# lior1990/hp-vae-gan

Hardware: AMD Instinct MI355X
Metric: train iters/sec per pyramid scale, air_balloons 13f@144p (higher is better)
Workload: dtype f32

## Files before the change

hp-vae-gan_amd/csrc/conv_mfma.hip:

```cpp
#include "hpvg_common.h"
#include "hpvg_host.h"
#include "hpvg.h"
#include <stdlib.h>

namespace {

__device__ const float g_zero_word[16] = {0.f, 0.f, 0.f, 0.f, 0.f, 0.f, 0.f, 0.f, 0.f, 0.f, 0.f, 0.f, 0.f, 0.f, 0.f, 0.f};
constexpr long HPVG_ZERO_PLANE_FLOATS = 1L << 18;
__device__ float g_zero_plane[HPVG_ZERO_PLANE_FLOATS];

#ifdef HPVG_TRACE
__device__ unsigned long long g_trace[8192 * 4];
__device__ unsigned long long g_phase[8192 * 4];
#define HPVG_PH(i) { unsigned long long now_ = __builtin_readcyclecounter(); ph_a[i] += now_ - ph_t; ph_t = now_; }
#define HPVG_PH_INIT unsigned long long ph_t = __builtin_readcyclecounter(); unsigned long long ph_a[4] = {0, 0, 0, 0};
#define HPVG_PH_END if (threadIdx.x == 0) { for (int i_ = 0; i_ < 4; ++i_) g_phase[4 * blockIdx.x + i_] = ph_a[i_]; }
#define HPVG_TRACE_BEGIN unsigned long long tr_t0 = wall_clock64(); unsigned long long tr_c0 = __builtin_readcyclecounter();
#define HPVG_TRACE_END                                                              \
  if (threadIdx.x == 0 && blockIdx.x + gridDim.x * (blockIdx.y + gridDim.y * blockIdx.z) < 8192) { \
    unsigned long long* tr = g_trace + 4 * (blockIdx.x + gridDim.x * (blockIdx.y + gridDim.y * blockIdx.z)); \
    tr[0] = tr_t0;                                                                  \
    tr[1] = wall_clock64();                                                         \
    tr[2] = __builtin_amdgcn_s_getreg((31 << 11) | 4);                              \
    tr[3] = (__builtin_amdgcn_s_getreg((31 << 11) | 20) & 0xF) | ((__builtin_readcyclecounter() - tr_c0) << 8); \
// ... 655 lines not shown
#pragma unroll
            for (int nt = 0; nt < NT; ++nt) acc[jj][nt] = __builtin_amdgcn_mfma_f32_32x32x2f32(v, Bf[j][nt], acc[jj][nt], 0, 0, 0);
          }
        }
      }
    };
    load_chunk(av[0], bv[0], 0);
    for (int s0 = 0; s0 < ksteps; s0 += 2 * KC) {
      load_chunk(av[1], bv[1], s0 + KC);
      __builtin_amdgcn_sched_barrier(0);
      mma_chunk(av[0], bv[0], s0);
      __builtin_amdgcn_sched_barrier(0);
      load_chunk(av[0], bv[0], s0 + 2 * KC);
      __builtin_amdgcn_sched_barrier(0);
      mma_chunk(av[1], bv[1], s0 + KC);
      __builtin_amdgcn_sched_barrier(0);
    }
#pragma unroll
    for (int nt = 0; nt < NT; ++nt) {
      const int n = nt * 32 + l31;
      if (n < CO9) {
#pragma unroll
        for (int jj = 0; jj < JB; ++jj)
#pragma unroll
          for (int e = 0; e < 16; ++e) P[n * pitch + GP * grp + JB * ((e & 3) + 8 * (e >> 2) + 4 * half) + jj] = acc[jj][nt][e];
      }
    }
  }
  __syncthreads();

  const int ob = g.ob[band], on = g.on[band];
  const int nout = g.Th * on;
  for (int idx = tid; idx < nout; idx += 256) {
    const int hh = idx / on, cc = idx - hh * on;
    const int gh = h0 + hh, gw = ob + cc;
    if (gh >= a.H) continue;
    const long sp = (long)t * HW + (long)gh * a.W + gw;
    for (int o = 0; o < a.Cout; ++o) {
      float v = 0.f;
#pragma unroll
      for (int dh = 0; dh < 3; ++dh)
#pragma unroll
        for (int dw = 0; dw < 3; ++dw) {
          const int gwt = gw + dw - 1;
          if (gwt >= 0 && gwt < a.W) v += P[(o * 9 + dh * 3 + dw) * pitch + (hh + dh) * RS + (gwt - wsb)];
        }
      if (a.bias) v += a.bias[o];
      if (a.out_lrelu) v = hpvg_lrelu(v);
      a.y[((long)b * a.Cout + o) * a.T * HW + sp] = v;
    }
  }
}

__global__ void conv_pack_narrow_kernel(const float* __restrict__ w, const float* __restrict__ inv_scale, float* __restrict__ wn,
                                        int Cin_k, int Cout_k, int KT, int NT, int ksteps, int transpose_flip, long total) {
  const long idx = (long)blockIdx.x * blockDim.x + threadIdx.x;
  if (idx >= total) return;
  const int lane = idx & 63;
  long r = idx >> 6;
  const int nt = r % NT;
  const int s = (int)(r / NT);
  const int k = (lane >> 5) * ksteps + s;
  const int n = nt * 32 + (lane & 31);
  const int c = k / KT, dt = k - c * KT;
  const int o = n / 9, tap = dt * 9 + (n - o * 9);
  const int taps = KT * 9;
  float val = 0.f;
  if (o < Cout_k && c < Cin_k) {
    if (!transpose_flip) val = w[((long)o * Cin_k + c) * taps + tap];
    else val = w[((long)c * Cout_k + o) * taps + (taps - 1 - tap)];
    if (inv_scale) val *= inv_scale[0];
  }
  wn[idx] = val;
}

__global__ void conv_pack_kernel(const float* __restrict__ w, const float* __restrict__ inv_scale, float* __restrict__ wp,
                                 int Cin_k, int Cout_k, int taps, int CC, int nchunk, int mbtot, int transpose_flip,
                                 long total_direct, long total) {
  const long idx = (long)blockIdx.x * blockDim.x + threadIdx.x;
  if (idx >= total) return;
  if (idx >= total_direct) {
    const long iw = idx - total_direct;
    const long nw1 = ((long)((Cin_k + WINO_CC - 1) / WINO_CC) * (taps / 9) * 3 * 4 + 4) * mbtot * 64 * (WINO_CC / 2);
    float val = iw < nw1 ? wino_pack_value(w, iw, Cin_k, Cout_k, taps / 9, (Cin_k + WINO_CC - 1) / WINO_CC, mbtot, transpose_flip)
                         : wino2_pack_value(w, iw - nw1, Cin_k, Cout_k, (Cin_k + 3) / 4, 2 * ((mbtot + 1) / 2), transpose_flip);
    if (inv_scale) val *= inv_scale[0];
    wp[idx] = val;
    return;
  }
  const int CP = CC / 2;
  long r = idx;
  const int cp = r % CP; r /= CP;
  const int lane = r % 64; r /= 64;
  const int mb = r % mbtot; r /= mbtot;
  const int tap = r % taps; r /= taps;
  const int ch = (int)r;
  float val = 0.f;
  if (ch < nchunk) {
    const int o = mb * 32 + (lane & 31);
    const int c = ch * CC + 2 * cp + (lane >> 5);
    if (o < Cout_k && c < Cin_k) {
      if (!transpose_flip) val = w[((long)o * Cin_k + c) * taps + tap];
      else val = w[((long)c * Cout_k + o) * taps + (taps - 1 - tap)];
      if (inv_scale) val *= inv_scale[0];
    }
  }
  wp[idx] = val;
}

struct PackBatchArgs {
  const float* w[HPVG_PACK_BATCH_MAX];
  float* wp[HPVG_PACK_BATCH_MAX];
  int flip[HPVG_PACK_BATCH_MAX];
};
__global__ void conv_pack_batch_kernel(const PackBatchArgs a, int C, int taps, int CC, int nchunk, int mbtot, long total_direct,
                                       long total) {
  const long idx = (long)blockIdx.x * blockDim.x + threadIdx.x;
  if (idx >= total) return;
  const int it = blockIdx.y;
  const float* __restrict__ w = a.w[it];
  const int transpose_flip = a.flip[it];
  if (idx >= total_direct) {
    const long iw = idx - total_direct;
    const long nw1 = ((long)((C + WINO_CC - 1) / WINO_CC) * (taps / 9) * 3 * 4 + 4) * mbtot * 64 * (WINO_CC / 2);
    a.wp[it][idx] = iw < nw1 ? wino_pack_value(w, iw, C, C, taps / 9, (C + WINO_CC - 1) / WINO_CC, mbtot, transpose_flip)
                             : wino2_pack_value(w, iw - nw1, C, C, (C + 3) / 4, 2 * ((mbtot + 1) / 2), transpose_flip);
    return;
  }
  const int CP = CC / 2;
  long r = idx;
  const int cp = r % CP; r /= CP;
  const int lane = r % 64; r /= 64;
  const int mb = r % mbtot; r /= mbtot;
  const int tap = r % taps; r /= taps;
  const int ch = (int)r;
  float val = 0.f;
  if (ch < nchunk) {
    const int o = mb * 32 + (lane & 31);
    const int c = ch * CC + 2 * cp + (lane >> 5);
    if (o < C && c < C) {
      if (!transpose_flip) val = w[((long)o * C + c) * taps + tap];
      else val = w[((long)c * C + o) * taps + (taps - 1 - tap)];
    }
  }
  a.wp[it][idx] = val;
}

struct CShape { int B, Cin, Cout, T, H, W, KT; };
inline int conv_check(const CShape& c) {
  if (c.B < 1 || c.Cin < 1 || c.Cout < 1 || c.T < 1 || c.H < 1 || c.W < 1) return HPVG_ERR_ARG;
  return c.KT == 1 || c.KT == 3 ? HPVG_OK : HPVG_ERR_UNSUPPORTED;
}

struct CKnobs {
  bool sk_off;
  bool narrow2_off;
  bool w2r;
  bool w2d_off;
  bool w2_split_off;
  int stagger;
  int only_nb, only_mb, only_ntw;
  int env_wino;
  int wino;
  long min_pos;
  int stg;
  int w2d;
  int gen;
};
CKnobs& cknobs() {
  static CKnobs knobs = [] {
    auto num = [](const char* name, long dflt) { const char* e = getenv(name); return e ? atol(e) : dflt; };
    CKnobs k{};
    k.sk_off = num("HPVG_CONV_SK", 1) == 0;
    k.narrow2_off = num("HPVG_NARROW2", 1) == 0;
    k.w2r = num("HPVG_WINO2R", 1) != 0;
    k.w2d_off = num("HPVG_WINO2D", 1) == 0;
    k.w2_split_off = num("HPVG_W2_SPLIT", 1) == 0;
    k.stagger = (int)num("HPVG_WINO_STAGGER", 0);
    k.only_nb = (int)num("HPVG_PLAN_NB", 0);
    k.only_mb = (int)num("HPVG_PLAN_MB", 0);
    k.only_ntw = (int)num("HPVG_PLAN_NTW", 0);
    k.wino = k.env_wino = (int)num("HPVG_WINO", 1);
    k.min_pos = num("HPVG_WINO_MIN", -1);
    const long stg = num("HPVG_WINO_STG", 0);
    k.stg = stg == 1 || stg == 2 ? (int)stg : 0;
    return k;
  }();
  return knobs;
}

inline int conv_cc(int Cin) { return Cin <= 4 ? 4 : 8; }
inline bool conv_is_narrow(int Cin, int Cout) { return Cout <= 4 && Cin > 4; }
inline bool conv_is_wino(const CKnobs& k, int Cin, int Cout) { return k.env_wino != 0 && Cin >= 8 && Cout > 32; }
inline bool conv_is_wino2d(const CKnobs& k, int Cin, int Cout, int KT) { return !k.w2d_off && KT == 3 && conv_is_wino(k, Cin, Cout); }

inline size_t direct_pack_floats(int Cin, int Cout, int KT) {
  const int CC = conv_cc(Cin);
  const int nchunk = hpvg_cdiv(Cin, CC);
  const int mbtot = hpvg_cdiv(Cout, 32);
  const size_t per_tap = (size_t)mbtot * 64 * (CC / 2);
  return ((size_t)nchunk * KT * 9 + 2) * per_tap;
}
size_t wpack_floats(int Cin, int Cout, int KT, bool with2d) {
  const CKnobs& k = cknobs();
  if (conv_is_narrow(Cin, Cout)) return (size_t)hpvg_cdiv(Cin * KT, 2) * hpvg_cdiv(9 * Cout, 32) * 64;
  return direct_pack_floats(Cin, Cout, KT) + (conv_is_wino(k, Cin, Cout) ? wino_pack_floats(Cin, Cout, KT) : 0) +
         (with2d && conv_is_wino2d(k, Cin, Cout, KT) ? wino2_pack_floats(Cin, Cout) : 0);
}

struct Plan {
  int Th, Tw, RS, PL, L, qstride, nrange, ntw, nblocks, NB, MB, gridy, nj;
  size_t lds;
  int stg;
};

constexpr long CONV_SLOTS = 2L * HPVG_NUM_CU;
inline long conv_slots(int MB, int NB) { return (long)HPVG_CONV_WGS(MB, NB) * HPVG_NUM_CU; }

inline double conv_cost(bool streamk, long ntl, int nchunk, long slots, double mfma_paired, double mfma_alone, double stage_us,
                        int blocks) {
  if (!streamk) {
    const long per_cu = (ntl + HPVG_NUM_CU - 1) / HPVG_NUM_CU;
    const double tile_paired = nchunk * (mfma_paired + 6.0 + stage_us) + 0.4 * blocks;
    const double tile_alone = nchunk * (mfma_alone + 2.0 + stage_us) + 0.4 * blocks;
    return (double)(per_cu / 2) * tile_paired + (double)(per_cu & 1) * tile_alone + 1e-4 * (double)ntl;
  }
  const long items_tot = ntl * nchunk;
// ... 193 lines not shown
  const int GP = 32 * JB;
  double best = 1e300;
  bool found = false;
  auto bands = [&](int RS, Narrow2Geom* q) -> int {
    int nb = 0, o = 0;
    while (o < W) {
      if (nb == 16) return 0;
      int n, ws;
      if (nb == 0) { n = (RS == W) ? W : RS - 1; ws = 0; }
      else if (W - o <= RS - 1) { n = W - o; ws = W - RS; }
      else { n = RS - 2; ws = o - 1; }
      if (n < 1) return 0;
      if (q) { q->ws[nb] = ws; q->ob[nb] = o; q->on[nb] = n; }
      o += n;
      ++nb;
    }
    return nb;
  };
  for (int RS = 4; RS <= 256 && RS <= W; RS += 4) {
    const int nb = bands(RS, nullptr);
    if (nb == 0) continue;
    for (int Th = 1; Th <= H; ++Th) {
      const int nth = hpvg_cdiv(H, Th);
      if (Th != hpvg_cdiv(H, nth)) continue;
      const int npos = (Th + 2) * RS;
      const int G = hpvg_cdiv(npos, GP);
      if (G > 16) break;
      const int pitch = (G * GP) | 1;
      if ((size_t)(9 * Cout) * pitch * sizeof(float) > 76 * 1024) break;
      const long nt = (long)B * T * nth * nb;
      const double rounds = hpvg_cdiv(G, 4);
      const double waves = nt <= 2L * HPVG_NUM_CU ? 1.0 : (double)nt / (2.0 * HPVG_NUM_CU);
      const double cost = waves * (rounds * GP + 30.0);
      if (cost < best) {
        best = cost;
        found = true;
        Narrow2Geom q{};
        q.RS = RS; q.Th = Th; q.nth = nth; q.nb = nb; q.npos = npos; q.G = G; q.pitch = pitch;
        bands(RS, &q);
        *out = q;
        *ntiles = nt;
      }
    }
  }
  if (!found) return false;
  for (int k = 0; k < out->nb; ++k) {
    const int lo = out->ob[k] - 1 < 0 ? 0 : out->ob[k] - 1;
    const int hi = out->ob[k] + out->on[k] > W - 1 ? W - 1 : out->ob[k] + out->on[k];
    if (out->on[k] < 0 || lo < out->ws[k] || hi >= out->ws[k] + out->RS) return false;
  }
  return true;
}

struct CPlans {
  Plan direct[2], wino[2];
  W2Geom w2;
  Narrow2Geom n2;
  long n2_tiles;
  bool n2_ok;
};
const CPlans& conv_plans(const CKnobs& k, const CShape& c) {
  return memo_lookup<CPlans>(k.gen, c.B, c.Cin, c.Cout, c.T, c.H, c.W, c.KT, [&] {
    CPlans pl{};
    if (conv_is_narrow(c.Cin, c.Cout)) {
      pl.direct[0] = pl.direct[1] = plan_narrow_search(c);
      pl.n2_ok = plan_narrow2(c.B, c.Cin, c.Cout, c.T, c.H, c.W, c.KT, &pl.n2, &pl.n2_tiles);
      return pl;
    }
    for (int sk = 0; sk < 2; ++sk) {
      pl.direct[sk] = plan_conv_search(k, c, sk != 0);
      if (conv_is_wino(k, c.Cin, c.Cout)) pl.wino[sk] = plan_wino_search(k, c, sk != 0);
    }
    pl.w2 = wino2d_geom(k, c);
    return pl;
  });
}

inline int conv_ntiles(const CShape& c, const Plan& p) { return c.B * c.T * p.nrange * p.ntw * p.gridy; }
inline int conv_sk_grid(const CShape& c, const Plan& p) {
  const long items = (long)conv_ntiles(c, p) * hpvg_cdiv(c.Cin, conv_cc(c.Cin));
  const long slots = conv_slots(p.MB, p.NB);
  return (int)(items < slots ? items : slots);
}
inline size_t conv_sk_ws_bytes(const CShape& c, const Plan& p) {
  return p.L ? (size_t)conv_sk_grid(c, p) * 2 * p.MB * p.NB * 16 * 256 * sizeof(float) : 0;
}

inline bool conv_use_wino(const CKnobs& k, const CShape& c, bool prologue) {
  if (prologue || !conv_is_wino(k, c.Cin, c.Cout) || k.wino == 0) return false;
  if (k.wino == 2) return true;
  const long min_pos = k.min_pos >= 0 ? k.min_pos : (c.KT == 3 ? 0L : 24000L);
  return (long)c.B * c.T * c.H * c.W >= min_pos;
}
inline bool conv_use_wino2d(const CKnobs& k, const W2Geom& q) {
  if (!q.ok || k.w2d == 1) return false;
  if (k.w2d == 2) return true;
  const long rounds = (q.ntl + HPVG_NUM_CU - 1) / HPVG_NUM_CU;
  if (rounds == 1) return q.ntl * 2 >= HPVG_NUM_CU;
  return (long)q.ntl * 10 >= 6L * rounds * HPVG_NUM_CU;
}

struct CDecision {
  int kind;
  int narrow_gen;
  const CPlans* plans;
  const Plan* plan;
  bool streamk;
  int ntl, S;
  size_t ws_bytes;
};
CDecision conv_decide(const CShape& c, bool prologue, bool fp32_out_mask, const void* ws, size_t ws_bytes) {
  const CKnobs& k = cknobs();
  CDecision d{};
  const CPlans& pl = conv_plans(k, c);
  d.plans = &pl;
  if (conv_is_narrow(c.Cin, c.Cout)) {
    d.kind = 3;
    d.plan = &pl.direct[0];
    d.narrow_gen = !k.narrow2_off && !prologue && !fp32_out_mask && pl.n2_ok ? 2 : 1;
    d.ntl = d.S = conv_ntiles(c, *d.plan);
    return d;
  }
  bool wino = conv_use_wino(k, c, prologue);
  if (wino && conv_use_wino2d(k, pl.w2) && !fp32_out_mask) {
    d.kind = 2;
    d.ntl = pl.w2.ntl;
    d.S = d.ntl < HPVG_NUM_CU ? d.ntl : HPVG_NUM_CU;
    return d;
  }
  d.streamk = !k.sk_off && ws != nullptr;
  if (wino && pl.wino[d.streamk].L == 0) wino = false;
  const Plan* both = wino ? pl.wino : pl.direct;
  if (d.streamk && ws_bytes < conv_sk_ws_bytes(c, both[1])) d.streamk = false;
  d.kind = wino ? 1 : 0;
  d.plan = &both[d.streamk];
  d.ntl = conv_ntiles(c, *d.plan);
  d.S = d.streamk ? conv_sk_grid(c, *d.plan) : d.ntl;
  d.ws_bytes = d.streamk ? conv_sk_ws_bytes(c, *d.plan) : 0;
  return d;
}
inline CDecision conv_decide_query(const CShape& c) { return conv_decide(c, false, false, &c, ~(size_t)0); }

struct CCall {
  const float* x; const float* wp; const float* bias;
  const float* in_scale; const float* in_shift; int in_lrelu;
  float* y; int out_lrelu;
  const float* out_mask; const unsigned* mask_bits; unsigned* bits_out;
  void* ws; size_t ws_bytes;
  CShape c;
  hipStream_t s;
};

ConvFwdArgs conv_args(const CCall& q, const CDecision& d, int stagger) {
  const CShape& c = q.c;
  const Plan& p = *d.plan;
  ConvFwdArgs a{};
  a.x = q.x; a.bias = q.bias; a.in_scale = q.in_scale; a.in_shift = q.in_shift; a.mask = q.out_mask; a.y = q.y;
  a.wp = d.kind == 1 ? q.wp + direct_pack_floats(c.Cin, c.Cout, c.KT) : q.wp;
  a.mask_bits = q.mask_bits; a.bits_out = q.bits_out;
  a.B = c.B; a.Cin = c.Cin; a.Cout = c.Cout; a.T = c.T; a.H = c.H; a.W = c.W;
  a.Th = p.Th; a.Tw = p.Tw; a.RS = p.RS; a.PL = p.PL; a.L = p.L; a.qstride = p.qstride; a.nrange = p.nrange; a.ntw = p.ntw; a.nblocks = p.nblocks;
  a.nchunk = hpvg_cdiv(c.Cin, conv_cc(c.Cin));
  a.mbtot = hpvg_cdiv(c.Cout, 32);
  a.nj = p.nj;
  a.in_lrelu = q.in_lrelu; a.out_lrelu = q.out_lrelu;
  a.gridy = p.gridy;
  a.ntl = d.ntl;
  a.ndp = d.ntl / d.S;
  a.skbase = a.ndp * d.S;
  a.skpart = d.kind == 3 ? nullptr : (float*)q.ws;
  a.stagger = d.kind == 1 && d.S > HPVG_NUM_CU ? stagger : 0;
  return a;
// ... 42 lines not shown
  const int rc = launch_lds<conv_wino_kernel<KT, WINO_NBP, VAR, STG>>(dim3(S), dim3(256), p.lds < CONV_MIN_LDS ? CONV_MIN_LDS : p.lds, s, a);
  const int nsk = a.ntl - a.skbase;
  if (rc != HPVG_OK || nsk <= 0) return rc;
  hipLaunchKernelGGL(conv_wino_fixup_kernel, dim3(nsk, WINO_NBP * 2), dim3(256), 0, s, a, S, WINO_NBP);
  return hpvg_launch_status();
}
template <int KT, int STG>
int launch_wino_stg(const ConvFwdArgs& a, const Plan& p, int S, hipStream_t s) {
  if (a.mask || a.mask_bits) return launch_wino_var<KT, VAR_MASK, STG>(a, p, S, s);
  if (a.bits_out) return launch_wino_var<KT, VAR_BITS, STG>(a, p, S, s);
  return launch_wino_var<KT, VAR_PLAIN, STG>(a, p, S, s);
}
template <int KT>
int launch_wino(const ConvFwdArgs& a, const Plan& p, int S, hipStream_t s) {
  return p.stg == 2 ? launch_wino_stg<KT, 2>(a, p, S, s) : launch_wino_stg<KT, 1>(a, p, S, s);
}

template <int VAR, bool TAIL, bool ODD>
int launch_wino2r_sub(int sub, const Wino2Args& a, int S, size_t lds, hipStream_t s) {
  if (sub == 2) return launch_lds<conv_wino2r_kernel<VAR, TAIL, ODD, 2>>(dim3(S), dim3(256), lds, s, a);
  if (sub == 1) return launch_lds<conv_wino2r_kernel<VAR, TAIL, ODD, 1>>(dim3(S), dim3(256), lds, s, a);
  return launch_lds<conv_wino2r_kernel<VAR, TAIL, ODD, 0>>(dim3(S), dim3(256), lds, s, a);
}
template <int VAR, bool TAIL>
int launch_wino2d_inst(bool w2r, int sub, const Wino2Args& a, int S, hipStream_t s) {
  const size_t lds = (size_t)3 * 12 * W2_PL * sizeof(float);
  if (a.W & 1) return launch_wino2r_sub<VAR, TAIL, true>(sub, a, S, lds, s);
  if (w2r) return launch_wino2r_sub<VAR, TAIL, false>(sub, a, S, lds, s);
  return launch_lds<conv_wino2d_kernel<VAR, TAIL>>(dim3(S), dim3(256), lds, s, a);
}
template <int VAR>
int launch_wino2d_var(bool w2r, int sub, const Wino2Args& a, int S, hipStream_t s) {
  return (((long)a.H * a.W) & 3) ? launch_wino2d_inst<VAR, true>(w2r, sub, a, S, s) : launch_wino2d_inst<VAR, false>(w2r, sub, a, S, s);
}
int launch_wino2d_form(bool w2r, int sub, const Wino2Args& a, int S, hipStream_t s) {
  if (a.mask_bits) return launch_wino2d_var<VAR_MASK>(w2r, sub, a, S, s);
  if (a.bits_out) return launch_wino2d_var<VAR_BITS>(w2r, sub, a, S, s);
  return launch_wino2d_var<VAR_PLAIN>(w2r, sub, a, S, s);
}
int launch_wino2d(bool w2r, Wino2Args a, const W2Geom& g, int S, hipStream_t s) {
  if (g.sp_parts == 1) return launch_wino2d_form(w2r, 0, a, S, s);
  a.ntl = g.sp_full;
  const int rc = launch_wino2d_form(w2r, 0, a, HPVG_NUM_CU, s);
  if (rc != HPVG_OK) return rc;
  a.sub0 = g.sp_full;
  a.ntl = g.sp_wgs;
  return launch_wino2d_form(w2r, g.sp_parts == 4 ? 2 : 1, a, g.sp_wgs, s);
}

template <int KT>
int launch_narrow(const ConvFwdArgs& a, const CDecision& d, hipStream_t s) {
  const int ksteps = hpvg_cdiv(a.Cin * KT, 2);
  const bool one = 9 * a.Cout <= 32;
  if (d.narrow_gen == 2) {
    const Narrow2Geom& g = d.plans->n2;
    const dim3 grid((unsigned)d.plans->n2_tiles);
    const size_t lds = (size_t)(9 * a.Cout) * g.pitch * sizeof(float);
    return one ? launch_lds<conv_narrow2_kernel<KT, 1, 4>>(grid, dim3(256), lds, s, a, g, ksteps)
               : launch_lds<conv_narrow2_kernel<KT, 2, 2>>(grid, dim3(256), lds, s, a, g, ksteps);
  }
  const int pitch = (hpvg_cdiv((d.plan->Th + 2) * d.plan->RS, 32) * 32) | 1;
  const size_t lds = (size_t)(9 * a.Cout) * pitch * sizeof(float);
  return one ? launch_lds<conv_narrow_kernel<KT, 1>>(dim3(a.ntl), dim3(256), lds, s, a, ksteps, pitch)
             : launch_lds<conv_narrow_kernel<KT, 2>>(dim3(a.ntl), dim3(256), lds, s, a, ksteps, pitch);
}

int conv_fwd_launch(const CCall& q) {
  const CShape& c = q.c;
  if (!q.x || !q.wp || !q.y) return HPVG_ERR_ARG;
  if (const int rc = conv_check(c)) return rc;
  if ((q.in_scale == nullptr) != (q.in_shift == nullptr)) return HPVG_ERR_ARG;
  if (q.in_scale && q.out_mask && !conv_is_narrow(c.Cin, c.Cout)) return HPVG_ERR_UNSUPPORTED;
  const CDecision d = conv_decide(c, q.in_scale != nullptr, q.out_mask != nullptr, q.ws, q.ws_bytes);
  if (d.kind == 2) return launch_wino2d(cknobs().w2r, wino2_args(q, d.plans->w2), d.plans->w2, d.S, q.s);
  if (d.plan->L == 0) return HPVG_ERR_UNSUPPORTED;
  const ConvFwdArgs a = conv_args(q, d, cknobs().stagger);
  if (d.kind == 3) return c.KT == 3 ? launch_narrow<3>(a, d, q.s) : launch_narrow<1>(a, d, q.s);
  if (d.kind == 1) return c.KT == 3 ? launch_wino<3>(a, *d.plan, d.S, q.s) : launch_wino<1>(a, *d.plan, d.S, q.s);
  if (conv_cc(c.Cin) == 8) return c.KT == 3 ? launch_conv<8, 3>(a, *d.plan, d.S, q.s) : launch_conv<8, 1>(a, *d.plan, d.S, q.s);
  return c.KT == 3 ? launch_conv<4, 3>(a, *d.plan, d.S, q.s) : launch_conv<4, 1>(a, *d.plan, d.S, q.s);
}

bool wants_wino2d(const CShape& c) { return conv_check(c) == HPVG_OK && conv_decide_query(c).kind == 2; }

int pack_weight_launch(const float* w, const float* inv_scale, float* wp, int Cin_layer, int Cout_layer, int KT, int transpose_flip,
                       bool with2d, void* stream) {
  if (!w || !wp || (KT != 1 && KT != 3) || Cin_layer < 1 || Cout_layer < 1) return HPVG_ERR_ARG;
  const int Cin_k = transpose_flip ? Cout_layer : Cin_layer;
  const int Cout_k = transpose_flip ? Cin_layer : Cout_layer;
  const long total = (long)wpack_floats(Cin_k, Cout_k, KT, with2d);
  if (conv_is_narrow(Cin_k, Cout_k)) {
    hipLaunchKernelGGL(conv_pack_narrow_kernel, dim3(hpvg_cdiv(total, 256)), dim3(256), 0, (hipStream_t)stream, w, inv_scale, wp,
                       Cin_k, Cout_k, KT, hpvg_cdiv(9 * Cout_k, 32), hpvg_cdiv(Cin_k * KT, 2), transpose_flip, total);
    return hpvg_launch_status();
  }
  const int CC = conv_cc(Cin_k);
  hipLaunchKernelGGL(conv_pack_kernel, dim3(hpvg_cdiv(total, 256)), dim3(256), 0, (hipStream_t)stream, w, inv_scale, wp, Cin_k, Cout_k,
                     KT * 9, CC, hpvg_cdiv(Cin_k, CC), hpvg_cdiv(Cout_k, 32), transpose_flip, (long)direct_pack_floats(Cin_k, Cout_k, KT),
                     total);
  return hpvg_launch_status();
}

int pack_batch_launch(int n, const float* const* w, float* const* wp, const int* flip, int C, int KT, bool with2d, void* stream) {
  if (n < 1 || n > HPVG_PACK_BATCH_MAX || !w || !wp || !flip || C <= 4 || (KT != 1 && KT != 3)) return HPVG_ERR_ARG;
  PackBatchArgs a;
  for (int i = 0; i < n; ++i) {
// ... 74 lines not shown

int hpvg_conv_fwd_plan(int B, int Cin, int Cout, int T, int H, int W, int KT, int* out) {
  const CShape c{B, Cin, Cout, T, H, W, KT};
  if (!out || conv_check(c) != HPVG_OK) return HPVG_ERR_ARG;
  const Plan& p = conv_plans(cknobs(), c).direct[1];
  return write_plan(p, p.nblocks, B * T * p.nrange * p.ntw, out);
}

int hpvg_conv_w2_split(int B, int Cin, int Cout, int T, int H, int W, int KT, int* out) {
  const CShape c{B, Cin, Cout, T, H, W, KT};
  if (!out || conv_check(c) != HPVG_OK) return HPVG_ERR_ARG;
  const CDecision d = conv_decide_query(c);
  if (d.kind != 2) return HPVG_ERR_UNSUPPORTED;
  const W2Geom& g = d.plans->w2;
  out[0] = g.sp_full; out[1] = g.ntl - g.sp_full; out[2] = g.sp_parts; out[3] = g.sp_wgs;
  return HPVG_OK;
}

int hpvg_conv_wino_config(int mode, long min_positions) {
  CKnobs& k = cknobs();
  if (k.env_wino == 0) return HPVG_ERR_UNSUPPORTED;
  if (mode >= 0) {
    const int stg = mode == 3 ? 2 : (mode == 4 ? 1 : 0);
    if (stg != k.stg) ++k.gen;
    k.wino = mode > 2 ? 2 : mode;
    k.stg = stg;
    k.w2d = mode == 5 ? 2 : (mode == 3 || mode == 4 || mode == 6 ? 1 : 0);
  }
  if (min_positions >= 0) k.min_pos = min_positions;
  if (k.wino == 2 && k.w2d == 2) return 5;
  if (k.wino == 2 && k.stg) return k.stg == 2 ? 3 : 4;
  if (k.wino == 2 && k.w2d == 1) return 6;
  return k.wino;
}

int hpvg_conv_wino_plan(int B, int Cin, int Cout, int T, int H, int W, int KT, int* out) {
  const CShape c{B, Cin, Cout, T, H, W, KT};
  if (!out || conv_check(c) != HPVG_OK) return HPVG_ERR_ARG;
  const Plan& p = conv_plans(cknobs(), c).wino[1];
  return p.L ? write_plan(p, p.RS, conv_ntiles(c, p), out) : HPVG_ERR_UNSUPPORTED;
}

int hpvg_conv_narrow_plan(int B, int Cin, int Cout, int T, int H, int W, int KT, int* out) {
  const CShape c{B, Cin, Cout, T, H, W, KT};
  if (!out || conv_check(c) != HPVG_OK) return HPVG_ERR_ARG;
  const CPlans& pl = conv_plans(cknobs(), c);
  if (!pl.n2_ok) return HPVG_ERR_UNSUPPORTED;
  const Narrow2Geom& g = pl.n2;
  out[0] = g.RS; out[1] = g.Th; out[2] = g.nth; out[3] = g.nb; out[4] = g.npos; out[5] = g.G; out[6] = g.pitch;
  for (int k = 0; k < g.nb; ++k) { out[7 + 3 * k] = g.ws[k]; out[8 + 3 * k] = g.ob[k]; out[9 + 3 * k] = g.on[k]; }
  return HPVG_OK;
}

#ifdef HPVG_TRACE
int hpvg_debug_phase_read(unsigned long long* host_out, int n) {
  return hipMemcpyFromSymbol(host_out, HIP_SYMBOL(g_phase), sizeof(unsigned long long) * 4 * n) == hipSuccess ? 0 : -4;
}
int hpvg_debug_trace_read(unsigned long long* host_out, int n) {
  return hipMemcpyFromSymbol(host_out, HIP_SYMBOL(g_trace), sizeof(unsigned long long) * 4 * n) == hipSuccess ? 0 : -4;
}
#endif

}
```

hp-vae-gan_amd/ops.py:

```python
import ctypes
import os

import torch
from torch.autograd import Function
from torch.autograd.function import once_differentiable

from .lib import PACK_BATCH_MAX, SN_BATCH_MAX, call, load, ptr, stream

_ws_cache = {}
_kernel_timer = None


class KernelTimer:

    def __init__(self, match):
        self.match = match
        self.events = []

    def begin(self, desc):
        fam = self.match(desc)
        if not fam:
            return None
        e0 = torch.cuda.Event(enable_timing=True)
        e0.record()
# ... 214 lines not shown

def conv_bwd_weight_bias_raw(dy, x, w_shape, into_w, into_b):
    dy = _c(dy)
    x = _c(x)
    B, Co, T, H, W = geom(dy)
    Ci = x.shape[1]
    KT = _kt(w_shape)
    if load().hpvg_conv_bwd_weight_fuses_bias(B, Ci, Co, T, H, W, KT) != 1:
        return False
    ws = _scratch(call("hpvg_conv_bwd_weight_ws_bytes", B, Ci, Co, T, H, W, KT), dy.device)
    timed = _kernel_timer.begin({"op": "wgrad", "Cin": Ci, "Cout": Co, "KT": KT, "bias": True}) if _kernel_timer is not None else None
    call("hpvg_conv_bwd_weight_bias_f32", ptr(dy), ptr(x), ptr(into_w), 1, ptr(into_b), 1, *ws, B, Ci, Co, T, H, W, KT, stream())
    if timed is not None:
        _kernel_timer.end(timed, (B, Ci, Co, T, H, W))
    return True


def channel_sum_raw(dy, into=None):
    dy = _c(dy)
    B, C, T, H, W = geom(dy)
    out = into if into is not None else torch.empty(C, dtype=torch.float32, device=dy.device)
    call("hpvg_channel_sum_f32", ptr(dy), ptr(out), 1 if into is not None else 0,
         *_scratch(call("hpvg_channel_sum_ws_bytes", C), dy.device), B, C, T * H * W, stream())
    return None if into is not None else out


def _weight_grad(dy, x, w):
    slot = grad_slot(w)
    if slot is not None:
        return conv_bwd_weight_raw(dy, x, w.shape, into=slot)
    return ConvBwdWeight.apply(dy, x, w.shape)


def _scalar_out(device):
    return torch.empty(1, dtype=torch.float32, device=device)


def _reduce_ws(device):
    n = call("hpvg_reduce_ws_bytes")
    return ptr(workspace(n, device)), n


class inputs_only:
    active = False

    def __enter__(self):
        self.prev = inputs_only.active
        inputs_only.active = True

    def __exit__(self, *exc):
        inputs_only.active = self.prev


class LReLUMaskMul(Function):

    @staticmethod
    def forward(ctx, dy, h):
        dy = _c(dy)
        out = torch.empty_like(dy)
        call("hpvg_lrelu_mask_mul_f32", ptr(dy), ptr(h), ptr(out), dy.numel(), stream())
        ctx.save_for_backward(h)
        return out

    @staticmethod
    def backward(ctx, g):
        (h,) = ctx.saved_tensors
        return LReLUMaskMul.apply(g, h), None


class ChannelSum(Function):
    @staticmethod
    def forward(ctx, dy):
        ctx.shape = dy.shape
        return channel_sum_raw(dy)

    @staticmethod
    def backward(ctx, g):
        view = [1, -1] + [1] * (len(ctx.shape) - 2)
        return g.view(*view).expand(ctx.shape).contiguous()


class Conv(Function):

    @staticmethod
    def forward(ctx, x, w, b, act, in_act=False, mask_by_consumer=False, in_bits=None):
        want = act and mask_by_consumer and w.shape[0] > 4
        if want:
            y, bits = conv_fwd_raw(x, w, b, out_lrelu=True, want_bits=True)
            Conv.last_bits = bits
        else:
            y = conv_fwd_raw(x, w, b, out_lrelu=act)
            Conv.last_bits = None
        own_mask = act and not mask_by_consumer
        ctx.save_for_backward(x, w, y if own_mask else None, b, in_bits if in_act else None)
        ctx.own_mask, ctx.in_act = own_mask, in_act
        ctx.has_bias = b is not None
        return y

    last_bits = None

    @staticmethod
    def apply_bits(x, w, b, act, in_act=False, mask_by_consumer=False, in_bits=None):
        y = Conv.apply(x, w, b, act, in_act, mask_by_consumer, in_bits)
        bits, Conv.last_bits = Conv.last_bits, None
        return y, bits

    @staticmethod
    def backward(ctx, dy):
        x, w, y, b, in_bits = ctx.saved_tensors
        dy = _c(dy)
        if ctx.own_mask:
            dy = LReLUMaskMul.apply(dy, y)
        params = not inputs_only.active
        dx = ConvBwdData.apply(dy, w, x if ctx.in_act else None, in_bits) if ctx.needs_input_grad[0] else None
        want_w = ctx.needs_input_grad[1] and params
        want_b = ctx.has_bias and ctx.needs_input_grad[2] and params
        if want_w and want_b:
            ws_, bs_ = grad_slot(w), grad_slot(b)
            if ws_ is not None and bs_ is not None and conv_bwd_weight_bias_raw(dy, x, w.shape, ws_, bs_):
                return dx, None, None, None, None, None, None
        dw = _weight_grad(dy, x, w) if want_w else None
        db = None
        if want_b:
            slot = grad_slot(b)
            db = channel_sum_raw(dy, into=slot) if slot is not None else ChannelSum.apply(dy)
        return dx, dw, db, None, None, None, None


class ConvBwdData(Function):

    @staticmethod
    def forward(ctx, dy, w, h=None, bits=None):
        ctx.save_for_backward(dy, w, h)
        if h is not None and bits is not None and w.shape[1] > 4:
            return conv_fwd_raw(dy, w, None, flip=True, mask_bits=bits)
        return conv_fwd_raw(dy, w, None, flip=True, out_mask=h)

    @staticmethod
    def backward(ctx, g):
        dy, w, h = ctx.saved_tensors
        g = _c(g)
        if h is not None:
            g = LReLUMaskMul.apply(g, h)
        ddy = Conv.apply(g, w, None, False) if ctx.needs_input_grad[0] else None
        dw = _weight_grad(dy, g, w) if ctx.needs_input_grad[1] else None
        return ddy, dw, None, None


class ConvBwdWeight(Function):

    @staticmethod
    def forward(ctx, dy, x, w_shape):
        ctx.save_for_backward(dy, x)
        return conv_bwd_weight_raw(dy, x, w_shape)

    @staticmethod
    def backward(ctx, gw):
        dy, x = ctx.saved_tensors
        gw = _c(gw)
        ddy = Conv.apply(x, gw, None, False) if ctx.needs_input_grad[0] else None
        dx = ConvBwdData.apply(dy, gw) if ctx.needs_input_grad[1] else None
        return ddy, dx, None


class BNAct(Function):

    @staticmethod
# ... 1180 lines not shown
```

include/hpvg.h:

```cpp
#ifndef HPVG_H
#define HPVG_H
#include <stddef.h>
#ifdef __cplusplus
extern "C" {
#endif

#define HPVG_OK 0
#define HPVG_ERR_ARG (-1)
#define HPVG_ERR_WORKSPACE (-2)
#define HPVG_ERR_UNSUPPORTED (-3)
#define HPVG_ERR_LAUNCH (-4)

size_t hpvg_conv_wpack_floats(int Cin, int Cout, int KT);
int hpvg_conv_pack_weight_f32(const float* w, const float* inv_scale, float* wp, int Cin_layer, int Cout_layer, int KT,
                              int transpose_flip, void* stream);
#define HPVG_PACK_BATCH_MAX 16
int hpvg_conv_pack_weight_batch_f32(int n, const float* const* w, float* const* wp, const int* flip, int C, int KT, void* stream);
size_t hpvg_conv_wpack_floats_for(int Cin, int Cout, int KT, int B, int T, int H, int W);
int hpvg_conv_wants_wino2d(int B, int Cin, int Cout, int T, int H, int W, int KT);
int hpvg_conv_pack_weight_for_f32(const float* w, const float* inv_scale, float* wp, int Cin_layer, int Cout_layer, int KT,
                                  int transpose_flip, int B, int T, int H, int W, void* stream);
int hpvg_conv_pack_weight_batch_for_f32(int n, const float* const* w, float* const* wp, const int* flip, int C, int KT, int B, int T,
                                        int H, int W, void* stream);
size_t hpvg_conv_fwd_ws_bytes(int B, int Cin, int Cout, int T, int H, int W, int KT);
int hpvg_conv_fwd_f32(const float* x, const float* wp, const float* bias, const float* in_scale, const float* in_shift,
                      int in_lrelu, float* y, int out_lrelu, const float* out_mask, void* ws, size_t ws_bytes, int B, int Cin,
                      int Cout, int T, int H, int W, int KT, void* stream);
size_t hpvg_conv_mask_words(int B, int C, int T, int H, int W);
int hpvg_conv_fwd_bits_f32(const float* x, const float* wp, const float* bias, float* y, int out_lrelu, const unsigned* mask_bits,
                           unsigned* bits_out, void* ws, size_t ws_bytes, int B, int Cin, int Cout, int T, int H, int W, int KT,
                           void* stream);
int hpvg_conv_fwd_plan(int B, int Cin, int Cout, int T, int H, int W, int KT, int* out10);
int hpvg_conv_fwd_kernel_kind(int B, int Cin, int Cout, int T, int H, int W, int KT);
int hpvg_conv_w2_split(int B, int Cin, int Cout, int T, int H, int W, int KT, int* out4);
int hpvg_conv_wino_config(int mode, long min_positions);
int hpvg_conv_wino_plan(int B, int Cin, int Cout, int T, int H, int W, int KT, int* out10);
int hpvg_conv_narrow_plan(int B, int Cin, int Cout, int T, int H, int W, int KT, int* out55);
size_t hpvg_conv_bwd_weight_ws_bytes(int B, int Cin, int Cout, int T, int H, int W, int KT);
int hpvg_conv_bwd_weight_f32(const float* dy, const float* x, const float* in_scale, const float* in_shift, int in_lrelu,
                             float* dw, int accumulate, void* ws, size_t ws_bytes, int B, int Cin, int Cout, int T, int H,
                             int W, int KT, void* stream);
int hpvg_conv_bwd_weight_plan(int B, int Cin, int Cout, int T, int H, int W, int KT, int* out10);
int hpvg_conv_bwd_weight_kernel_kind(int B, int Cin, int Cout, int T, int H, int W, int KT);
int hpvg_conv_bwd_weight_wino_config(int mode);
int hpvg_conv_bwd_weight_fuses_bias(int B, int Cin, int Cout, int T, int H, int W, int KT);
int hpvg_conv_bwd_weight_bias_f32(const float* dy, const float* x, float* dw, int accumulate, float* db, int accumulate_db, void* ws,
                                  size_t ws_bytes, int B, int Cin, int Cout, int T, int H, int W, int KT, void* stream);
int hpvg_conv_bwd_weight_wino_plan(int B, int Cin, int Cout, int T, int H, int W, int KT, int* out10);
int hpvg_conv_bwd_weight_wino2_plan(int B, int Cin, int Cout, int T, int H, int W, int KT, int* out11);
size_t hpvg_channel_sum_ws_bytes(int C);
int hpvg_channel_sum_f32(const float* x, float* out, int accumulate, void* ws, size_t ws_bytes, int B, int C, long S,
                         void* stream);

size_t hpvg_bn_ws_bytes(int C);
int hpvg_bn_train_stats_f32(const float* x, const float* gamma, const float* beta, float* running_mean, float* running_var,
                            float momentum, float eps, float* mean, float* invstd, float* scale, float* shift, void* ws,
                            size_t ws_bytes, int B, int C, long S, void* stream);
int hpvg_bn_train_fwd_f32(const float* x, const float* gamma, const float* beta, float* running_mean, float* running_var,
                          float momentum, float eps, float* mean, float* invstd, float* scale, float* shift, float* y, int lrelu,
                          int groups, void* ws, size_t ws_bytes, int B, int C, long S, void* stream);
int hpvg_affine_act_f32(const float* x, const float* scale, const float* shift, float* y, int lrelu, int B, int C, long S,
                        void* stream);
int hpvg_bn_act_bwd_f32(const float* dh, const float* r, const float* mean, const float* invstd, const float* scale,
                        const float* shift, int lrelu, int groups, float* dr, float* dgamma, float* dbeta, int accumulate, void* ws,
                        size_t ws_bytes, int B, int C, long S, void* stream);
int hpvg_bn_plan(int B, int C, long S, int groups, int* out3);
int hpvg_vec_width_at(const void* p, long S);
int hpvg_bn_vec_width_at(const void* p, int B, int C, long S, int groups);
size_t hpvg_bn_bwd2_ws_bytes(int C);
int hpvg_bn_act_bwd2_f32(const float* dh, const float* g, const float* r, const float* mean, const float* invstd, const float* scale,
                         const float* shift, int lrelu, float* g_dh, float* g_r, float* g_gamma, int accumulate, void* ws,
                         size_t ws_bytes, int B, int C, long S, void* stream);
int hpvg_bn_sums_f32(const float* x, double* sums, void* ws, size_t ws_bytes, int B, int C, long S, void* stream);
int hpvg_bn_finalize_f32(const double* sums, double count, const float* gamma, const float* beta, float* running_mean,
                         float* running_var, float momentum, float eps, float* mean, float* invstd, float* scale, float* shift,
                         int C, void* stream);
int hpvg_bn_act_bwd_sums_f32(const float* dh, const float* r, const float* mean, const float* invstd, const float* scale,
                             const float* shift, int lrelu, double* sums, void* ws, size_t ws_bytes, int B, int C, long S,
                             void* stream);
int hpvg_bn_act_bwd_apply_f32(const float* dh, const float* r, const float* mean, const float* invstd, const float* scale,
                              const float* shift, int lrelu, const float* sums, float inv_count, float* dr, int B, int C, long S,
                              void* stream);
int hpvg_lrelu_mask_mul_f32(const float* dy, const float* h, float* out, long n, void* stream);

int hpvg_add_f32(const float* a, const float* b, float* out, long n, void* stream);
int hpvg_copy_f32(const float* src, float* dst, long n, void* stream);
int hpvg_box_copy_f32(const float* src, float* dst, long BC, int sT, int sH, int sW, int dT, int dH, int dW, int oT, int oH,
                      int oW, void* stream);
int hpvg_tanh_fwd_f32(const float* x, const float* res , float* y, long n, void* stream);
int hpvg_tanh_bwd_f32(const float* dy, const float* y, float* dx, long n, void* stream);
// ... 124 lines not shown
```

Baseline: 32.28.

## Add temporal-rolling narrow conv kernel reusing input planes across output frames

Adds a new narrow-output (Cout<=4) 3D conv forward kernel. It loads each input time plane once and computes the partial products for all three temporal taps with MFMA into LDS. The results are accumulated into rolling register buffers and emitted one frame late, so input planes are not reloaded per output frame. It is selected by default for Cout==1, T>=7 with enough workgroups, and adds a planner over band and row-tile geometry. The Python backward also detaches the tensors used as masks, which avoids autograd bookkeeping but would drop double-backward through them.

```diff
diff --git a/hp-vae-gan_amd/csrc/conv_mfma.hip b/hp-vae-gan_amd/csrc/conv_mfma.hip
--- a/hp-vae-gan_amd/csrc/conv_mfma.hip
+++ b/hp-vae-gan_amd/csrc/conv_mfma.hip
@@ -731,6 +731,165 @@
   }
 }
 
+struct NarrowTGeom {
+  int RS, Th, nth, nb, npos, G, pitch;
+  int ws[16], ob[16], on[16];
+};
+constexpr int NARROWT_PPT = 4;
+constexpr size_t NARROWT_LDS_MAX = 76 * 1024;
+
+template <int COUT>
+__global__ __launch_bounds__(256, 2) void conv_narrowt_kernel(const ConvFwdArgs a, const NarrowTGeom g) {
+  typedef f32x4u AV;
+  constexpr int JB = 4, GP = 32 * JB, KC = 8, PPT = NARROWT_PPT;
+  constexpr int NTO = (9 * COUT + 31) / 32;
+  extern __shared__ __attribute__((aligned(16))) float P[];
+  const int tid = threadIdx.x;
+  const int lane = tid & 63;
+  const int wave = __builtin_amdgcn_readfirstlane(tid >> 6);
+  const int half = lane >> 5, l31 = lane & 31;
+  const long HW = (long)a.H * a.W;
+  const int RS = g.RS, pitch = g.pitch;
+  const int Ch = a.Cin >> 1;
+
+  int r = hpvg_xcd_remap(blockIdx.x, gridDim.x);
+  const int band = r % g.nb; r /= g.nb;
+  const int th = r % g.nth;
+  const int b = r / g.nth;
+  const int h0 = th * g.Th, wsb = g.ws[band], ob = g.ob[band], on = g.on[band];
+  const char* xb = reinterpret_cast<const char*>(a.x + (long)b * a.Cin * a.T * HW + wsb);
+  const unsigned lhalf = (unsigned)((long)half * Ch * a.T * HW);
+  const long cstep = a.T * HW * 4;
+
+  const int dtn = l31 < 27 ? l31 / 9 : 0, j9 = l31 < 27 ? l31 - 9 * dtn : 0;
+  int woff[COUT];
+#pragma unroll
+  for (int o = 0; o < COUT; ++o) woff[o] = (dtn * NTO + ((o * 9 + j9) >> 5)) * 64 + half * 32 + ((o * 9 + j9) & 31);
+  constexpr int wstep = 3 * NTO * 64;
+
+  const int nout = g.Th * on;
+  int ohh[PPT], occ[PPT];
+  bool own[PPT];
+  float rA[PPT][COUT], rB[PPT][COUT], rC[PPT][COUT];
+#pragma unroll
+  for (int p = 0; p < PPT; ++p) {
+    const int idx = tid + 256 * p;
+    const bool in = idx < nout;
+    ohh[p] = in ? idx / on : 0;
+    occ[p] = in ? idx - ohh[p] * on : 0;
+    own[p] = in && h0 + ohh[p] < a.H;
+#pragma unroll
+    for (int o = 0; o < COUT; ++o) rA[p][o] = rB[p][o] = rC[p][o] = 0.f;
+  }
+  auto store_plane = [&](const float (&rr)[PPT][COUT], int tau) {
+#pragma unroll
+    for (int p = 0; p < PPT; ++p) {
+      if (!own[p]) continue;
+      const long sp = (long)tau * HW + (long)(h0 + ohh[p]) * a.W + ob + occ[p];
+#pragma unroll
+      for (int o = 0; o < COUT; ++o) {
+        float v = rr[p][o];
+        if (a.bias) v += a.bias[o];
+        if (a.out_lrelu) v = hpvg_lrelu(v);
+        a.y[((long)b * COUT + o) * a.T * HW + sp] = v;
+      }
+    }
+  };
+
+  for (int t = 0; t < a.T; ++t) {
+#pragma unroll
+    for (int o = 0; o < COUT; ++o) {
+      const float* wq = a.wp + woff[o];
+      for (int grp = wave; grp < g.G; grp += 4) {
+        const int p = GP * grp + JB * l31;
+        const int pc = p < g.npos ? p : g.npos - JB;
+        const int row = pc / RS, col = pc - row * RS;
+        const int gh = h0 - 1 + row;
+        const bool valid = p < g.npos && gh >= 0 && gh < a.H;
+        const int ghc = gh < 0 ? 0 : (gh >= a.H ? a.H - 1 : gh);
+        const char* xt = xb + (long)t * HW * 4;
+        const unsigned lofs = (lhalf + (unsigned)(ghc * a.W + col)) * 4u;
+        f32x16 acc[JB];
+#pragma unroll
+        for (int j = 0; j < JB; ++j)
+#pragma unroll
+          for (int e = 0; e < 16; ++e) acc[j][e] = 0.f;
+        AV av[2][KC];
+        float bv[2][KC];
+        auto load_chunk = [&](AV (&A)[KC], float (&Bf)[KC], int s0) {
+#pragma unroll
+          for (int j = 0; j < KC; ++j) {
+            const int s = s0 + j;
+            if (s < Ch) {
+              A[j] = *reinterpret_cast<const AV*>(xt + s * cstep + lofs);
+              Bf[j] = wq[s * wstep];
+            }
+          }
+        };
+        auto mma_chunk = [&](const AV (&A)[KC], const float (&Bf)[KC], int s0) {
+#pragma unroll
+          for (int j = 0; j < KC; ++j) {
+            if (s0 + j < Ch) {
+#pragma unroll
+              for (int jj = 0; jj < JB; ++jj)
+                acc[jj] = __builtin_amdgcn_mfma_f32_32x32x2f32(valid ? A[j][jj] : 0.f, Bf[j], acc[jj], 0, 0, 0);
+            }
+          }
+        };
+        load_chunk(av[0], bv[0], 0);
+        for (int s0 = 0; s0 < Ch; s0 += 2 * KC) {
+          load_chunk(av[1], bv[1], s0 + KC);
+          __builtin_amdgcn_sched_barrier(0);
+          mma_chunk(av[0], bv[0], s0);
+          __builtin_amdgcn_sched_barrier(0);
+          load_chunk(av[0], bv[0], s0 + 2 * KC);
+          __builtin_amdgcn_sched_barrier(0);
+          mma_chunk(av[1], bv[1], s0 + KC);
+          __builtin_amdgcn_sched_barrier(0);
+        }
+        if (l31 < 27) {
+#pragma unroll
+          for (int jj = 0; jj < JB; ++jj)
+#pragma unroll
+            for (int e = 0; e < 16; ++e) P[l31 * pitch + GP * grp + JB * ((e & 3) + 8 * (e >> 2) + 4 * half) + jj] = acc[jj][e];
+        }
+      }
+      __syncthreads();
+#pragma unroll
+      for (int p = 0; p < PPT; ++p) {
+        if (!own[p]) continue;
+        int hh = ohh[p], cc = occ[p];
+        asm volatile("" : "+v"(hh), "+v"(cc));
+        const int gw = ob + cc;
+        const float* Pp = P + hh * RS + (gw - wsb);
+        float sdt[3];
+#pragma unroll
+        for (int dt = 0; dt < 3; ++dt) {
+          float v = 0.f;
+#pragma unroll
+          for (int dh = 0; dh < 3; ++dh)
+#pragma unroll
+            for (int dw = 0; dw < 3; ++dw) {
+              const int gwt = gw + dw - 1;
+              if (gwt >= 0 && gwt < a.W) v += Pp[(dt * 9 + dh * 3 + dw) * pitch + dh * RS + (dw - 1)];
+            }
+          sdt[dt] = v;
+        }
+        rC[p][o] = sdt[0];
+        rB[p][o] += sdt[1];
+        rA[p][o] += sdt[2];
+      }
+      __syncthreads();
+    }
+    if (t >= 1) store_plane(rA, t - 1);
+#pragma unroll
+    for (int p = 0; p < PPT; ++p)
+#pragma unroll
+      for (int o = 0; o < COUT; ++o) { rA[p][o] = rB[p][o]; rB[p][o] = rC[p][o]; }
+  }
+  store_plane(rA, a.T - 1);
+}
+
 __global__ void conv_pack_narrow_kernel(const float* __restrict__ w, const float* __restrict__ inv_scale, float* __restrict__ wn,
                                         int Cin_k, int Cout_k, int KT, int NT, int ksteps, int transpose_flip, long total) {
   const long idx = (long)blockIdx.x * blockDim.x + threadIdx.x;
@@ -834,6 +993,7 @@
 struct CKnobs {
   bool sk_off;
   bool narrow2_off;
+  int narrowt;
   bool w2r;
   bool w2d_off;
   bool w2_split_off;
@@ -852,6 +1012,8 @@
     CKnobs k{};
     k.sk_off = num("HPVG_CONV_SK", 1) == 0;
     k.narrow2_off = num("HPVG_NARROW2", 1) == 0;
+    const long nt = num("HPVG_NARROWT", 0);
+    k.narrowt = nt == 1 || nt == 2 ? (int)nt : 0;
     k.w2r = num("HPVG_WINO2R", 1) != 0;
     k.w2d_off = num("HPVG_WINO2D", 1) == 0;
     k.w2_split_off = num("HPVG_W2_SPLIT", 1) == 0;
@@ -1151,12 +1313,77 @@
   return true;
 }
 
+bool plan_narrowt(int B, int Cin, int Cout, int T, int H, int W, int KT, NarrowTGeom* out, long* nwg) {
+  if (KT != 3 || (Cin & 1) || Cin < 2 || Cout > 4 || W < 4) return false;
+  if ((long)Cin * T * H * W >= (1L << 30)) return false;
+  constexpr int GP = 128;
+  double best = 1e300;
+  bool found = false;
+  auto bands = [&](int RS, NarrowTGeom* q) -> int {
+    int nb = 0, o = 0;
+    while (o < W) {
+      if (nb == 16) return 0;
+      int n, ws;
+      if (nb == 0) { n = (RS == W) ? W : RS - 1; ws = 0; }
+      else if (W - o <= RS - 1) { n = W - o; ws = W - RS; }
+      else { n = RS - 2; ws = o - 1; }
+      if (n < 1) return 0;
+      if (q) { q->ws[nb] = ws; q->ob[nb] = o; q->on[nb] = n; }
+      o += n;
+      ++nb;
+    }
+    return nb;
+  };
+  for (int RS = 4; RS <= 256 && RS <= W; RS += 4) {
+    const int nb = bands(RS, nullptr);
+    if (nb == 0) continue;
+    const int on_max = RS == W ? W : RS - 1;
+    for (int Th = 1; Th <= H; ++Th) {
+      const int nth = hpvg_cdiv(H, Th);
+      if (Th != hpvg_cdiv(H, nth)) continue;
+      if (Th * on_max > 256 * NARROWT_PPT) break;
+      const int npos = (Th + 2) * RS;
+      const int G = hpvg_cdiv(npos, GP);
+      const int pitch = (G * GP) | 1;
+      if ((size_t)27 * pitch * sizeof(float) > NARROWT_LDS_MAX) break;
+      const long n = (long)B * nth * nb;
+      const double cost = (double)hpvg_cdiv(n, (long)HPVG_NUM_CU) * (hpvg_cdiv(G, 4) * GP + 40.0) + 1e-3 * (double)(n * G);
+      if (cost < best) {
+        best = cost;
+        found = true;
+        NarrowTGeom q{};
+        q.RS = RS; q.Th = Th; q.nth = nth; q.nb = nb; q.npos = npos; q.G = G; q.pitch = pitch;
+        bands(RS, &q);
+        *out = q;
+        *nwg = n;
+      }
+    }
+  }
+  if (!found) return false;
+  for (int k = 0; k < out->nb; ++k) {
+    const int lo = out->ob[k] - 1 < 0 ? 0 : out->ob[k] - 1;
+    const int hi = out->ob[k] + out->on[k] > W - 1 ? W - 1 : out->ob[k] + out->on[k];
+    if (out->on[k] < 1 || lo < out->ws[k] || hi >= out->ws[k] + out->RS) return false;
+    if (out->ws[k] < 0 || out->ws[k] + out->RS > W) return false;
+  }
+  return true;
+}
+inline size_t narrowt_lds(const NarrowTGeom& g) { return (size_t)27 * g.pitch * sizeof(float); }
+inline bool conv_use_narrowt(const CKnobs& k, const CShape& c, bool ok, long nwg) {
+  if (!ok || k.narrowt == 1) return false;
+  if (k.narrowt == 2) return true;
+  return c.Cout == 1 && c.T >= 7 && nwg >= 180;
+}
+
 struct CPlans {
   Plan direct[2], wino[2];
   W2Geom w2;
   Narrow2Geom n2;
   long n2_tiles;
   bool n2_ok;
+  NarrowTGeom nt;
+  long nt_wgs;
+  bool nt_ok;
 };
 const CPlans& conv_plans(const CKnobs& k, const CShape& c) {
   return memo_lookup<CPlans>(k.gen, c.B, c.Cin, c.Cout, c.T, c.H, c.W, c.KT, [&] {
@@ -1164,6 +1391,7 @@
     if (conv_is_narrow(c.Cin, c.Cout)) {
       pl.direct[0] = pl.direct[1] = plan_narrow_search(c);
       pl.n2_ok = plan_narrow2(c.B, c.Cin, c.Cout, c.T, c.H, c.W, c.KT, &pl.n2, &pl.n2_tiles);
+      pl.nt_ok = plan_narrowt(c.B, c.Cin, c.Cout, c.T, c.H, c.W, c.KT, &pl.nt, &pl.nt_wgs);
       return pl;
     }
     for (int sk = 0; sk < 2; ++sk) {
@@ -1217,6 +1445,7 @@
     d.kind = 3;
     d.plan = &pl.direct[0];
     d.narrow_gen = !k.narrow2_off && !prologue && !fp32_out_mask && pl.n2_ok ? 2 : 1;
+    if (!prologue && !fp32_out_mask && conv_use_narrowt(k, c, pl.nt_ok, pl.nt_wgs)) d.narrow_gen = 3;
     d.ntl = d.S = conv_ntiles(c, *d.plan);
     return d;
   }
@@ -1365,6 +1594,19 @@
 int launch_narrow(const ConvFwdArgs& a, const CDecision& d, hipStream_t s) {
   const int ksteps = hpvg_cdiv(a.Cin * KT, 2);
   const bool one = 9 * a.Cout <= 32;
+  if constexpr (KT == 3) {
+    if (d.narrow_gen == 3) {
+      const NarrowTGeom& g = d.plans->nt;
+      const dim3 grid((unsigned)d.plans->nt_wgs);
+      const size_t lds = narrowt_lds(g);
+      switch (a.Cout) {
+        case 1: return launch_lds<conv_narrowt_kernel<1>>(grid, dim3(256), lds, s, a, g);
+        case 2: return launch_lds<conv_narrowt_kernel<2>>(grid, dim3(256), lds, s, a, g);
+        case 3: return launch_lds<conv_narrowt_kernel<3>>(grid, dim3(256), lds, s, a, g);
+        default: return launch_lds<conv_narrowt_kernel<4>>(grid, dim3(256), lds, s, a, g);
+      }
+    }
+  }
   if (d.narrow_gen == 2) {
     const Narrow2Geom& g = d.plans->n2;
     const dim3 grid((unsigned)d.plans->n2_tiles);
@@ -1545,6 +1787,26 @@
   return HPVG_OK;
 }
 
+int hpvg_conv_narrowt_plan(int B, int Cin, int Cout, int T, int H, int W, int KT, int* out) {
+  const CShape c{B, Cin, Cout, T, H, W, KT};
+  if (!out || conv_check(c) != HPVG_OK) return HPVG_ERR_ARG;
+  const CPlans& pl = conv_plans(cknobs(), c);
+  if (!pl.nt_ok) return HPVG_ERR_UNSUPPORTED;
+  const NarrowTGeom& g = pl.nt;
+  out[0] = g.RS; out[1] = g.Th; out[2] = g.nth; out[3] = g.nb; out[4] = g.npos; out[5] = g.G; out[6] = g.pitch;
+  out[7] = (int)narrowt_lds(g);
+  out[8] = conv_decide_query(c).narrow_gen == 3 ? 1 : 0;
+  for (int k = 0; k < g.nb; ++k) { out[9 + 3 * k] = g.ws[k]; out[10 + 3 * k] = g.ob[k]; out[11 + 3 * k] = g.on[k]; }
+  return HPVG_OK;
+}
+
+int hpvg_conv_narrowt_config(int mode) {
+  CKnobs& k = cknobs();
+  if (mode > 2) return HPVG_ERR_ARG;
+  if (mode >= 0) k.narrowt = mode;
+  return k.narrowt;
+}
+
 #ifdef HPVG_TRACE
 int hpvg_debug_phase_read(unsigned long long* host_out, int n) {
   return hipMemcpyFromSymbol(host_out, HIP_SYMBOL(g_phase), sizeof(unsigned long long) * 4 * n) == hipSuccess ? 0 : -4;
diff --git a/hp-vae-gan_amd/ops.py b/hp-vae-gan_amd/ops.py
--- a/hp-vae-gan_amd/ops.py
+++ b/hp-vae-gan_amd/ops.py
@@ -290,6 +290,9 @@
         inputs_only.active = self.prev
 
 
+DETACH_MASKS = True
+
+
 class LReLUMaskMul(Function):
 
     @staticmethod
@@ -347,10 +350,14 @@
     def backward(ctx, dy):
         x, w, y, b, in_bits = ctx.saved_tensors
         dy = _c(dy)
+        if DETACH_MASKS:
+            x_mask, y_mask = x.detach(), (y.detach() if y is not None else None)
+        else:
+            x_mask, y_mask = x, y
         if ctx.own_mask:
-            dy = LReLUMaskMul.apply(dy, y)
+            dy = LReLUMaskMul.apply(dy, y_mask)
         params = not inputs_only.active
-        dx = ConvBwdData.apply(dy, w, x if ctx.in_act else None, in_bits) if ctx.needs_input_grad[0] else None
+        dx = ConvBwdData.apply(dy, w, x_mask if ctx.in_act else None, in_bits) if ctx.needs_input_grad[0] else None
         want_w = ctx.needs_input_grad[1] and params
         want_b = ctx.has_bias and ctx.needs_input_grad[2] and params
         if want_w and want_b:
diff --git a/include/hpvg.h b/include/hpvg.h
--- a/include/hpvg.h
+++ b/include/hpvg.h
@@ -36,6 +36,8 @@
 int hpvg_conv_wino_config(int mode, long min_positions);
 int hpvg_conv_wino_plan(int B, int Cin, int Cout, int T, int H, int W, int KT, int* out10);
 int hpvg_conv_narrow_plan(int B, int Cin, int Cout, int T, int H, int W, int KT, int* out55);
+int hpvg_conv_narrowt_plan(int B, int Cin, int Cout, int T, int H, int W, int KT, int* out57);
+int hpvg_conv_narrowt_config(int mode);
 size_t hpvg_conv_bwd_weight_ws_bytes(int B, int Cin, int Cout, int T, int H, int W, int KT);
 int hpvg_conv_bwd_weight_f32(const float* dy, const float* x, const float* in_scale, const float* in_shift, int in_lrelu,
                              float* dw, int accumulate, void* ws, size_t ws_bytes, int B, int Cin, int Cout, int T, int H,
```

New measurement: 34.56, median of 6. 7.1% higher.
